# HuttleyLab/DiverseSeq

Measured on NVIDIA B200. Metric: prep_nmost_throughput, higher is better.
Workload: dtype u8 bases -> u32 counts -> f64 frequencies/entropy/JSD

## Files before the change

### diverseseq_b200/csrc/count.cu

```cuda
#include <stdlib.h>

#include <algorithm>

#include <functional>

#include "comm.cuh"
#include "common.cuh"
#include "fused.cuh"
#include "entropy.cuh"

namespace dvs {

struct CountWork {
    uint64_t begin;
    uint64_t end;
    uint32_t rec;
    uint32_t part;
};

constexpr int kCountThreads = 512;
constexpr int kPrefetch = 4;

__device__ __forceinline__ uint32_t pack4(uint32_t w) {
    return (w * 0x40100401u) >> 24;
}
__device__ __forceinline__ uint32_t pack16(uint4 v) {
    return (pack4(v.x) << 24) | (pack4(v.y) << 16) | (pack4(v.z) << 8) | pack4(v.w);
}

__device__ __forceinline__ uint4 ldg16(const uint8_t* p) { return __ldg(reinterpret_cast<const uint4*>(p)); }

template <bool SMEM>
__global__ void __launch_bounds__(kCountThreads)
k_count_generic(const uint8_t* __restrict__ seqs, const uint64_t* __restrict__ offsets,
                const CountWork* __restrict__ work, uint32_t nwork, uint32_t* __restrict__ next_item, int k,
                uint32_t num_states, uint64_t dim, uint32_t part_bins, uint32_t* __restrict__ counts) {
    extern __shared__ uint32_t hist[];
    __shared__ uint32_t s_item;
    const int tid = threadIdx.x;
    for (;;) {
        if (tid == 0) s_item = atomicAdd(next_item, 1u);
        __syncthreads();
        const uint32_t item = s_item;
        if (item >= nwork) break;
        const CountWork w = work[item];
        const uint64_t start = offsets[w.rec], end = offsets[w.rec + 1];
        const uint32_t part_base = w.part * part_bins;
        uint32_t* grow = counts + (size_t)w.rec * dim;
        if (SMEM) {
            for (uint32_t i = tid; i < part_bins; i += kCountThreads) hist[i] = 0;
            __syncthreads();
        }
        for (uint64_t a = w.begin + (uint64_t)tid * 16; a < w.end; a += (uint64_t)kCountThreads * 16) {
            const uint4 cur = ldg16(seqs + a);
            const uint4 prev = ldg16(seqs + a - 16);
            const uint32_t wv[8] = {prev.x, prev.y, prev.z, prev.w, cur.x, cur.y, cur.z, cur.w};
            uint32_t run = 0;
            uint64_t idx = 0;
#pragma unroll
            for (int i = 0; i < 32; ++i) {
                const uint64_t p = a - 16 + i;
                uint32_t b = (wv[i >> 2] >> (8 * (i & 3))) & 0xFFu;
                if (p < start || p >= end) b = 0xFFu;
                if (b >= num_states) {
                    run = 0;
                    idx = 0;
                } else {
                    idx = (idx * num_states + b) % dim;
                    ++run;
                    if (i >= 16 && run >= (uint32_t)k) {
                        if (SMEM) {
                            uint32_t local = (uint32_t)idx - part_base;
                            if (local < part_bins) atomicAdd(&hist[local], 1u);
                        } else {
                            atomicAdd(&grow[idx], 1u);
                        }
                    }
                }
            }
        }
        if (SMEM) {
            __syncthreads();
            for (uint32_t i = tid; i < part_bins; i += kCountThreads) {
                uint32_t c = hist[i];
                if (c && (uint64_t)part_base + i < dim) atomicAdd(&grow[part_base + i], c);
            }
        }
        __syncthreads();
    }
}

constexpr int MODE_SMEM = 0, MODE_SMEM_PARTS = 1, MODE_GLOBAL = 2, MODE_SUPER = 3, MODE_SUPER3 = 4;

__device__ __forceinline__ uint32_t pack16p(uint4 v) {
    const uint32_t p0 = v.x * 0x40100401u, p1 = v.y * 0x40100401u, p2 = v.z * 0x40100401u, p3 = v.w * 0x40100401u;
    const uint32_t hi = __byte_perm(p1, p0, 0x7300);
    const uint32_t lo = __byte_perm(p3, p2, 0x0073);
    return __byte_perm(lo, hi, 0x7610);
}

__device__ __forceinline__ uint32_t scr_word(uint32_t idx) { return idx ^ (idx >> 5); }

template <int MODE, bool SCR, int THREADS>
__global__ void __launch_bounds__(THREADS)
k_count(const uint8_t* __restrict__ seqs, const uint64_t* __restrict__ offsets, const CountWork* __restrict__ work,
        uint32_t nwork, uint32_t* __restrict__ next_item, int k, uint64_t dim, uint32_t part_bins,
        uint32_t* __restrict__ counts, const uint32_t* __restrict__ nwork_dev) {
    extern __shared__ uint32_t hist[];
    __shared__ uint32_t s_item;
    if (nwork_dev) nwork = *nwork_dev;
    const int tid = threadIdx.x, lane = tid & 31, warp = tid >> 5;
    constexpr int kWarps = THREADS / 32;
    constexpr uint32_t kFull = 0xffffffffu;
    const int kk = (MODE == MODE_SUPER) ? k + 1 : k;
    const uint32_t mask = (kk >= 16) ? 0xFFFFFFFFu : ((1u << (2 * kk)) - 1u);
    const uint32_t mask4 = mask << 2;
    const uint32_t mask_k = (k >= 16) ? 0xFFFFFFFFu : ((1u << (2 * k)) - 1u);
    const uint32_t hist_words = (MODE == MODE_SUPER) ? (uint32_t)(dim * 4 + dim)
                                                     : (MODE == MODE_SMEM_PARTS ? part_bins + 1 : part_bins);
    uint32_t* side = hist + dim * 4;
    char* const hist_b = reinterpret_cast<char*>(hist);

    for (;;) {
        if (tid == 0) s_item = atomicAdd(next_item, 1u);
        __syncthreads();
        const uint32_t item = s_item;
        if (item >= nwork) break;
        const CountWork w = work[item];
        const uint64_t start = offsets[w.rec], end = offsets[w.rec + 1];
        const uint32_t part_base = (MODE == MODE_SMEM_PARTS) ? w.part * part_bins : 0u;
        uint32_t* grow = counts + (size_t)w.rec * dim;
        if (MODE != MODE_GLOBAL) {
            for (uint32_t i = tid; i < hist_words; i += THREADS) hist[i] = 0;
            __syncthreads();
        }
        auto bump4 = [&](uint32_t idx4) {
            if (MODE == MODE_SMEM || MODE == MODE_SUPER) {
                if (SCR) idx4 ^= (idx4 >> 5) & ~3u;
                atomicAdd(reinterpret_cast<uint32_t*>(hist_b + idx4), 1u);
            } else if (MODE == MODE_SMEM_PARTS) {
                uint32_t local4 = idx4 - (part_base << 2);
                if (SCR) local4 ^= (local4 >> 5) & ~3u;
                local4 = min(local4, part_bins << 2);
                atomicAdd(reinterpret_cast<uint32_t*>(hist_b + local4), 1u);
            } else {
                atomicAdd(&grow[idx4 >> 2], 1u);
            }
        };

        const uint32_t item_len = (uint32_t)(w.end - w.begin);
        const uint32_t rs = start > w.begin ? (uint32_t)min(start - w.begin, (uint64_t)item_len) : 0u;
        const uint32_t re = end < w.end ? (end > w.begin ? (uint32_t)(end - w.begin) : 0u) : item_len;
        const uint32_t span = ((item_len + kWarps - 1) / kWarps + 511u) & ~511u;
        const uint32_t r0 = min(item_len, (uint32_t)warp * span);
        const uint32_t r1 = min(item_len, r0 + span);
        const uint8_t* base = seqs + w.begin;
        uint32_t carry_pc = 0;
        bool carry_ok = false;
        uint4 ring[kPrefetch];
#pragma unroll
        for (int u = 0; u < kPrefetch; ++u) {
            const uint32_t a = r0 + 512u * u + 16 * lane;
            ring[u] = (a < r1) ? ldg16(base + a) : make_uint4(~0u, ~0u, ~0u, ~0u);
        }
        if (r0 < r1) {
            const uint4 h = ldg16(base + r0 - 16);
            const uint64_t a0 = w.begin + r0;
            carry_ok = (((h.x | h.y | h.z | h.w) & 0xFCFCFCFCu) == 0) && (a0 >= start + 16) && (a0 <= end);
            carry_pc = pack16p(h);
        }
        for (uint32_t rbase = r0; rbase < r1; rbase += 512u * kPrefetch) {
#pragma unroll
          for (int u = 0; u < kPrefetch; ++u) {
            const uint32_t r = rbase + 512u * u;
            if (r >= r1) break;
            const uint32_t a = r + 16 * lane;
            const uint4 cur = ring[u];
            ring[u] = (a + 512u * kPrefetch < r1) ? ldg16(base + a + 512u * kPrefetch) : make_uint4(~0u, ~0u, ~0u, ~0u);
            const bool ok = (((cur.x | cur.y | cur.z | cur.w) & 0xFCFCFCFCu) == 0) && (a >= rs) && (a + 16 <= re) && (a < r1);
            const uint32_t pc = pack16p(cur);
            uint32_t pp = __shfl_up_sync(kFull, pc, 1);
            if (lane == 0) pp = carry_pc;
            const uint32_t okmask = __ballot_sync(kFull, ok);
            const bool all_fast = (okmask == kFull) && carry_ok;
            if (all_fast) {
                if (MODE == MODE_SUPER) {
#pragma unroll
                    for (int j = 1; j < 15; j += 2) bump4(__funnelshift_r(pc, pp, 2 * (15 - j) - 2) & mask4);
                    bump4((pc << 2) & mask4);
                } else {
#pragma unroll
                    for (int j = 0; j < 15; ++j) bump4(__funnelshift_r(pc, pp, 2 * (15 - j) - 2) & mask4);
                    bump4((pc << 2) & mask4);
                }
            } else if (a < r1) {
                const bool prev_ok = lane == 0 ? carry_ok : ((okmask >> (lane - 1)) & 1u) != 0;
                if (ok && prev_ok) {
                    if (MODE == MODE_SUPER) {
#pragma unroll
                        for (int j = 1; j < 16; j += 2) bump4((__funnelshift_r(pc, pp, 2 * (15 - j)) & mask) << 2);
                    } else {
#pragma unroll
                        for (int j = 0; j < 16; ++j) bump4((__funnelshift_r(pc, pp, 2 * (15 - j)) & mask) << 2);
                    }
                } else {
                    const uint4 prev = ldg16(base + a - 16);
                    const uint32_t wv[8] = {prev.x, prev.y, prev.z, prev.w, cur.x, cur.y, cur.z, cur.w};
                    uint32_t run = 0, idx = 0, run_even = 0, idx_even = 0;
#pragma unroll
                    for (int i = 0; i < 32; ++i) {
                        const uint64_t p = w.begin + a + i - 16;
                        uint32_t bb = (wv[i >> 2] >> (8 * (i & 3))) & 0xFFu;
                        if (p < start || p >= end) bb = 0xFFu;
                        if (bb >= 4u) {
                            run = 0;
                            idx = 0;
                        } else {
                            idx = ((idx << 2) | bb) & mask;
                            ++run;
                        }
                        if (i < 16) continue;
                        if (MODE != MODE_SUPER) {
                            if (run >= (uint32_t)k) bump4(idx << 2);
                        } else if ((i & 1) == 0) {
                            run_even = run;
                            idx_even = idx;
                        } else if (run >= (uint32_t)(k + 1)) {
                            bump4(idx << 2);
                        } else {
                            if (run_even >= (uint32_t)k) atomicAdd(&side[idx_even & mask_k], 1u);
                            if (run >= (uint32_t)k) atomicAdd(&side[idx & mask_k], 1u);
                        }
                    }
                }
            }
            carry_pc = __shfl_sync(kFull, pc, 31);
            carry_ok = (okmask >> 31) != 0;
          }
        }
        if (MODE != MODE_GLOBAL) {
            __syncthreads();
            if (MODE == MODE_SUPER) {
                for (uint32_t x = tid; x < (uint32_t)dim; x += THREADS) {
                    uint32_t c = side[x];
#pragma unroll
                    for (uint32_t b = 0; b < 4; ++b) {
                        const uint32_t y = (x << 2) | b;
                        c += hist[SCR ? scr_word(y) : y];
                    }
#pragma unroll
                    for (uint32_t a4 = 0; a4 < 4; ++a4) {
                        const uint32_t y = (a4 << (2 * k)) | x;
                        c += hist[SCR ? scr_word(y) : y];
                    }
                    if (c) atomicAdd(&grow[x], c);
                }
            } else {
                for (uint32_t i = tid; i < part_bins; i += THREADS) {
                    uint32_t c = hist[SCR ? scr_word(i) : i];
                    if (c && (uint64_t)part_base + i < dim) atomicAdd(&grow[part_base + i], c);
                }
            }
        }
        __syncthreads();
    }
}

__device__ __forceinline__ void ldg32(const uint8_t* p, uint32_t (&v)[8]) {
    asm volatile("ld.global.nc.v8.u32 {%0,%1,%2,%3,%4,%5,%6,%7}, [%8];"
                 : "=r"(v[0]), "=r"(v[1]), "=r"(v[2]), "=r"(v[3]), "=r"(v[4]), "=r"(v[5]), "=r"(v[6]), "=r"(v[7])
                 : "l"(p));
}
__device__ __forceinline__ uint32_t pack16w(uint32_t x, uint32_t y, uint32_t z, uint32_t w) {
    return pack16p(make_uint4(x, y, z, w));
}

template <bool SCR, int THREADS, int PF>
__device__ __forceinline__ void
count_s3_body(const uint8_t* __restrict__ seqs, const uint64_t* __restrict__ offsets, const CountWork* __restrict__ work,
           uint32_t nwork, uint32_t* __restrict__ next_item, int k, uint64_t dim, uint32_t* __restrict__ counts,
           CountWork* __restrict__ retry, uint32_t* __restrict__ retry_count, uint32_t* resident) {
    extern __shared__ uint32_t hist[];
    __shared__ uint32_t s_item, s_sum, s_inc;
    if (resident && threadIdx.x == 0) atomicAdd(resident, 1u);
    const int tid = threadIdx.x, lane = tid & 31, warp = tid >> 5;
    constexpr int kWarps = THREADS / 32;
    constexpr uint32_t kFull = 0xffffffffu, kStep = 1024u;
    const int kk = k + 2;
    const uint32_t mask = (1u << (2 * kk)) - 1u;
    const uint32_t mask_k = (1u << (2 * k)) - 1u;
    const uint32_t hwords = (uint32_t)(dim * 8);
    uint32_t* side = hist + hwords;
    char* const hist_b = reinterpret_cast<char*>(hist);
    char* const side_b = reinterpret_cast<char*>(side);
    const uint32_t offmask = mask << 1 & ~3u, sidemask4 = mask_k << 2;
    const uint32_t lane32 = 32u * (uint32_t)lane;

    for (;;) {
        if (tid == 0) {
            s_item = atomicAdd(next_item, 1u);
            s_sum = 0;
            s_inc = 0;
        }
        __syncthreads();
        const uint32_t item = s_item;
        if (item >= nwork) break;
        const CountWork w = work[item];
        const uint64_t start = offsets[w.rec], end = offsets[w.rec + 1];
        uint32_t* grow = counts + (size_t)w.rec * dim;
        {
            uint4* h4 = reinterpret_cast<uint4*>(hist);
            const uint32_t n4 = (hwords + (uint32_t)dim) / 4;
            for (uint32_t i = tid; i < n4; i += THREADS) h4[i] = make_uint4(0, 0, 0, 0);
        }
        __syncthreads();
        uint32_t n_fast = 0;
        auto bump_v = [&](uint32_t v) {
            uint32_t off = v & offmask;
            if (SCR) off ^= (off >> 5) & ~3u;
            atomicAdd(reinterpret_cast<uint32_t*>(hist_b + off), (v & 2u) ? 0x10000u : 1u);
        };
        auto fast_block = [&](uint32_t pc, uint32_t pp) {
#pragma unroll
            for (int t = 0; t < 5; ++t) bump_v(__funnelshift_r(pc, pp, 25 - 6 * t));
            atomicAdd(reinterpret_cast<uint32_t*>(side_b + ((pc << 2) & sidemask4)), 1u);
        };

        const uint32_t item_len = (uint32_t)(w.end - w.begin);
        const uint32_t rs = start > w.begin ? (uint32_t)min(start - w.begin, (uint64_t)item_len) : 0u;
        const uint32_t re = end < w.end ? (end > w.begin ? (uint32_t)(end - w.begin) : 0u) : item_len;
        const uint32_t span = ((item_len + kWarps - 1) / kWarps + kStep - 1u) & ~(kStep - 1u);
        const uint32_t r0 = min(item_len, (uint32_t)warp * span);
        const uint32_t r1 = min(item_len, r0 + span);
        const uint8_t* base = seqs + w.begin;
        const uint32_t safe_hi = min(re, r1);
        uint32_t carry_pc = 0;
        bool carry_ok = false;
        uint32_t ring[PF][8];
#pragma unroll
        for (int u = 0; u < PF; ++u) {
            const uint32_t a = r0 + kStep * u + lane32;
            if (a < r1) ldg32(base + a, ring[u]);
            else {
#pragma unroll
                for (int q = 0; q < 8; ++q) ring[u][q] = ~0u;
            }
        }
        if (r0 < r1) {
            const uint4 h = ldg16(base + r0 - 16);
            const uint64_t a0 = w.begin + r0;
            carry_ok = (((h.x | h.y | h.z | h.w) & 0xFCFCFCFCu) == 0) && (a0 >= start + 16) && (a0 <= end);
            carry_pc = pack16p(h);
        }
        for (uint32_t rbase = r0; rbase < r1; rbase += kStep * PF) {
#pragma unroll
          for (int u = 0; u < PF; ++u) {
            const uint32_t r = rbase + kStep * u;
            if (r >= r1) break;
            const uint32_t a = r + lane32;
            uint32_t any = ring[u][0] | ring[u][1] | ring[u][2] | ring[u][3] | ring[u][4] | ring[u][5] | ring[u][6] | ring[u][7];
            bool ok = (any & 0xFCFCFCFCu) == 0;
            if (!(r >= rs && r + kStep <= safe_hi)) ok = ok && (a >= rs) && (a + 32 <= safe_hi);
            const uint32_t pc0 = pack16w(ring[u][0], ring[u][1], ring[u][2], ring[u][3]);
            const uint32_t pc1 = pack16w(ring[u][4], ring[u][5], ring[u][6], ring[u][7]);
            {
                const uint32_t an = a + kStep * PF;
                if (an < r1) ldg32(base + an, ring[u]);
                else {
#pragma unroll
                    for (int q = 0; q < 8; ++q) ring[u][q] = ~0u;
                }
            }
            uint32_t pp0 = __shfl_up_sync(kFull, pc1, 1);
            if (lane == 0) pp0 = carry_pc;
            const uint32_t okmask = __ballot_sync(kFull, ok);
            bool fast = okmask == kFull && carry_ok;
            if (!fast) {
                const bool prev_ok = lane == 0 ? carry_ok : ((okmask >> (lane - 1)) & 1u) != 0;
                fast = ok && prev_ok;
            }
            if (fast) {
                fast_block(pc0, pp0);
                fast_block(pc1, pc0);
                n_fast += 2;
            } else if (a < r1) {
                const uint4 q0 = ldg16(base + a - 16), q1 = ldg16(base + a), q2 = ldg16(base + a + 16);
                const uint32_t wv[12] = {q0.x, q0.y, q0.z, q0.w, q1.x, q1.y, q1.z, q1.w, q2.x, q2.y, q2.z, q2.w};
                uint32_t run = 0, idx = 0;
#pragma unroll 4
                for (int i = 0; i < 48; ++i) {
                    const uint64_t p = w.begin + a + i - 16;
                    uint32_t bb = (wv[i >> 2] >> (8 * (i & 3))) & 0xFFu;
                    if (p < start || p >= end) bb = 0xFFu;
                    if (bb >= 4u) {
                        run = 0;
                        idx = 0;
                    } else {
                        idx = ((idx << 2) | bb) & mask_k;
                        ++run;
                        if (i >= 16 && a + i - 16 < r1 && run >= (uint32_t)k) atomicAdd(&side[idx], 1u);
                    }
                }
            }
            carry_pc = __shfl_sync(kFull, pc1, 31);
            carry_ok = (okmask >> 31) != 0;
          }
        }
        __syncthreads();
        uint32_t pre_sum = 0;
        auto word_at = [&](uint32_t wd) { return hist[SCR ? (wd ^ (wd >> 5)) : wd]; };
        for (uint32_t x = tid; x < (uint32_t)dim; x += THREADS) {
            uint32_t c = side[x], pre = 0;
#pragma unroll
            for (uint32_t t = 0; t < 8; ++t) {
                const uint32_t v = word_at((x << 3) | t);
                pre += (v & 0xFFFFu) + (v >> 16);
            }
            c += pre;
            pre_sum += pre;
#pragma unroll
            for (uint32_t a4 = 0; a4 < 4; ++a4) {
#pragma unroll
                for (uint32_t t = 0; t < 2; ++t) {
                    const uint32_t v = word_at((a4 << (2 * k + 1)) | (x << 1) | t);
                    c += (v & 0xFFFFu) + (v >> 16);
                }
            }
#pragma unroll
            for (uint32_t t = 0; t < 16; ++t) {
                const uint32_t v = word_at((t << (2 * k - 1)) | (x >> 1));
                c += (x & 1u) ? (v >> 16) : (v & 0xFFFFu);
            }
            side[x] = c;
        }
        uint32_t n_inc = 5u * n_fast;
#pragma unroll
        for (int o = 16; o; o >>= 1) {
            pre_sum += __shfl_xor_sync(kFull, pre_sum, o);
            n_inc += __shfl_xor_sync(kFull, n_inc, o);
        }
        if (lane == 0) {
            atomicAdd(&s_sum, pre_sum);
            atomicAdd(&s_inc, n_inc);
        }
        __syncthreads();
        if (s_sum == s_inc) {
            for (uint32_t x = tid; x < (uint32_t)dim; x += THREADS) {
                const uint32_t c = side[x];
                if (c) atomicAdd(&grow[x], c);
            }
        } else if (tid == 0) {
            retry[atomicAdd(retry_count, 1u)] = w;
        }
        __syncthreads();
    }
    if (resident && threadIdx.x == 0) atomicSub(resident, 1u);
}

template <bool SCR, int THREADS, int PF>
__global__ void __launch_bounds__(THREADS, 1)
k_count_s3(const uint8_t* __restrict__ seqs, const uint64_t* __restrict__ offsets, const CountWork* __restrict__ work,
           uint32_t nwork, uint32_t* __restrict__ next_item, int k, uint64_t dim, uint32_t* __restrict__ counts,
           CountWork* __restrict__ retry, uint32_t* __restrict__ retry_count) {
    count_s3_body<SCR, THREADS, PF>(seqs, offsets, work, nwork, next_item, k, dim, counts, retry, retry_count, nullptr);
}
template <int MAXR>
__global__ void __maxnreg__(MAXR)
k_count_s3_trail(const uint8_t* __restrict__ seqs, const uint64_t* __restrict__ offsets,
                 const CountWork* __restrict__ work, uint32_t nwork, uint32_t* __restrict__ next_item, int k,
                 uint64_t dim, uint32_t* __restrict__ counts, CountWork* __restrict__ retry,
                 uint32_t* __restrict__ retry_count, uint32_t* resident) {
    count_s3_body<false, 1024, 2>(seqs, offsets, work, nwork, next_item, k, dim, counts, retry, retry_count, resident);
}

__global__ void __launch_bounds__(kEntThreads)
k_freq_entropy(const uint32_t* __restrict__ counts, uint64_t dim, double* __restrict__ freqs,
               uint64_t* __restrict__ totals, double* __restrict__ entropy, uint8_t* __restrict__ valid,
               uint8_t* __restrict__ err, double* __restrict__ err_total, const uint32_t* __restrict__ rec_list) {
    extern __shared__ __align__(16) double ent_smem[];
    __shared__ unsigned long long s_total;
    const uint32_t r = rec_list ? rec_list[blockIdx.x] : blockIdx.x;
    const uint32_t* c = counts + (size_t)r * dim;
    double* f = freqs + (size_t)r * dim;
    if (threadIdx.x == 0) s_total = 0ULL;
    __syncthreads();
    unsigned long long part = 0;
    for (uint64_t i = threadIdx.x; i < dim; i += blockDim.x) part += c[i];
    for (int o = 16; o; o >>= 1) part += __shfl_xor_sync(0xffffffffu, part, o);
    if ((threadIdx.x & 31) == 0) atomicAdd(&s_total, part);
    __syncthreads();
    const unsigned long long total_u = s_total;
    const double total = (double)total_u;
    if (total_u == 0ULL) {
        for (uint64_t i = threadIdx.x; i < dim; i += blockDim.x) f[i] = __ddiv_rn((double)c[i], total);
        if (threadIdx.x == 0) {
            totals[r] = 0;
            entropy[r] = 0.0;
            valid[r] = 0;
            err[r] = 0;
            err_total[r] = 0.0;
        }
        return;
    }
    const FastDiv dv = make_fast_div(total);
    EntropyResult h = block_entropy_exact(dim, [&](uint64_t i) {
        const double x = div_exact((double)c[i], dv);
        f[i] = x;
        return x;
    }, ent_smem);
    if (threadIdx.x == 0) {
        totals[r] = total_u;
        entropy[r] = h.e;
        valid[r] = 1;
        bool bad = entropy_total_bad(h.t, dim);
        err[r] = bad ? 1 : 0;
        err_total[r] = h.t;
    }
}

__global__ void __launch_bounds__(kEntThreads)
k_rows_entropy(const double* __restrict__ freqs, uint64_t dim, double* __restrict__ entropy,
               uint8_t* __restrict__ err, double* __restrict__ err_total, int write_entropy) {
    extern __shared__ __align__(16) double ent_smem[];
    const uint32_t r = blockIdx.x;
    const double* f = freqs + (size_t)r * dim;
    EntropyResult h = block_entropy_exact(dim, [&](uint64_t i) { return f[i]; }, ent_smem);
    if (threadIdx.x == 0) {
        if (write_entropy) entropy[r] = h.e;
        bool bad = entropy_total_bad(h.t, dim);
        err[r] = bad ? 1 : 0;
        err_total[r] = h.t;
    }
}

__global__ void k_take_rows(const double* __restrict__ F, const double* __restrict__ H, const uint8_t* __restrict__ V,
                            const uint8_t* __restrict__ E, const double* __restrict__ ET, uint64_t dim,
                            const uint32_t* __restrict__ rows, double* __restrict__ Fo, double* __restrict__ Ho,
                            uint8_t* __restrict__ Vo, uint8_t* __restrict__ Eo, double* __restrict__ ETo) {
    const uint32_t i = blockIdx.x, r = rows[i];
    const double* src = F + (size_t)r * dim;
    double* dst = Fo + (size_t)i * dim;
    for (uint64_t c = threadIdx.x; c < dim; c += blockDim.x) dst[c] = src[c];
    if (threadIdx.x == 0) {
        Ho[i] = H[r];
        Vo[i] = V[r];
        Eo[i] = E[r];
        ETo[i] = ET[r];
    }
}

__global__ void k_log2(const double* x, double* y, uint64_t n) {
    uint64_t i = (uint64_t)blockIdx.x * blockDim.x + threadIdx.x;
    if (i < n) y[i] = dvs_log2(x[i]);
}

static bool pow_dim(int num_states, int k, uint64_t* dim) {
    uint64_t d = 1;
    for (int i = 0; i < k; ++i) {
        d *= (uint64_t)num_states;
        if (d > (1ULL << 32)) return false;
    }
    *dim = d;
    return true;
}

static int kfreqs_alloc(dvs_ctx* ctx, uint32_t nrec, uint64_t dim, bool with_counts, dvs_kfreqs** out) {
    DVS_CUDA_TRY(dvs::enter(ctx));
    auto* f = new dvs_kfreqs();
    f->device = ctx->device;
    f->nrec = nrec;
    f->dim = dim;
    f->has_counts = with_counts;
    int rc = DVS_OK;
    if (with_counts) rc = f->counts.alloc((size_t)nrec * dim);
    if (rc == DVS_OK) rc = f->freqs.alloc((size_t)nrec * dim);
    if (rc == DVS_OK) rc = f->totals.alloc(nrec);
    if (rc == DVS_OK) rc = f->entropy.alloc(nrec);
    if (rc == DVS_OK) rc = f->valid.alloc(nrec);
    if (rc == DVS_OK) rc = f->err.alloc(nrec);
    if (rc == DVS_OK) rc = f->err_total.alloc(nrec);
    if (rc != DVS_OK) {
        delete f;
        return rc;
    }
    *out = f;
    return DVS_OK;
}

}

using namespace dvs;

extern "C" {

struct CountDest {
    double* freqs;
    uint64_t* totals;
    double* entropy;
    uint8_t* valid;
    uint8_t* err;
    double* err_total;
    uint32_t chunks;
    std::function<int(uint32_t, uint32_t)> after_chunk;
    const uint32_t* rec_seq = nullptr;
    int s3_shape = -1;
    uint32_t* resident = nullptr;
    int trail_regs = 56;
    const uint32_t* weights = nullptr;
};

static int count_core(dvs_ctx* ctx, const dvs_seqset* s, int k, int num_states, uint32_t* d_counts, uint64_t dim,
                      const CountDest& dst) {
    cudaStream_t st = ctx->stream;
#define TRY_F(expr)                                                          \
    do {                                                                     \
        cudaError_t _e = (expr);                                             \
        if (_e != cudaSuccess) {                                             \
            set_error("%s failed: %s", #expr, cudaGetErrorString(_e));       \
            return DVS_ERR_CUDA;                                             \
        }                                                                    \
    } while (0)

    TRY_F(cudaMemsetAsync(d_counts, 0, (size_t)s->nrec * dim * sizeof(uint32_t), st));

    const bool ns4 = (num_states == 4);
    const size_t max_hist_bytes = std::min<size_t>(ctx->smem_optin > 4096 ? ctx->smem_optin - 2048 : 0, 128 * 1024 + 16);
    uint32_t nparts = 1, part_bins = (uint32_t)std::min<uint64_t>(dim, 1u << 31);
    int mode = MODE_SMEM;
    size_t hist_bytes = (size_t)dim * 4;
    const char* s3_env = getenv("DVS_COUNT_S3");
    const bool want_s3 = !(s3_env && s3_env[0] == '0');
    if (ns4 && want_s3 && k >= 4 && dim * 36 + 2048 <= ctx->smem_optin && dim * 36 <= 160 * 1024) {
        mode = MODE_SUPER3;
        hist_bytes = (size_t)dim * 36;
    } else if (ns4 && dim * 20 <= 96 * 1024) {
        mode = MODE_SUPER;
        hist_bytes = (size_t)dim * 20;
    } else if (dim * 4 > max_hist_bytes) {
        uint64_t bins_per = max_hist_bytes / 4;
        uint64_t np = (dim + bins_per - 1) / bins_per;
        if (np <= 2) {
            mode = MODE_SMEM_PARTS;
            nparts = (uint32_t)np;
            part_bins = (uint32_t)((dim + np - 1) / np);
            hist_bytes = (size_t)part_bins * 4 + 16;
        } else {
            mode = MODE_GLOBAL;
            hist_bytes = 0;
        }
    }
    const bool smem = (mode != MODE_GLOBAL);
    const char* scr_env = getenv("DVS_COUNT_SCRAMBLE");
    const bool scramble = !(scr_env && scr_env[0] == '0');

    int ctas_per_sm = 4;
    if (smem) ctas_per_sm = (int)std::max<size_t>(1, std::min<size_t>(4, (ctx->smem_optin + 1024) / (hist_bytes + 1024)));
    const uint32_t grid = (uint32_t)(ctx->sm_count * ctas_per_sm);
    const int threads4 = (mode == MODE_SMEM_PARTS || mode == MODE_SUPER3) ? 1024 : kCountThreads;
    uint64_t chunk = 1 << 20;
    {
        const uint64_t flush_bins =
            (mode == MODE_GLOBAL) ? 0 : (mode == MODE_SUPER ? dim : (mode == MODE_SUPER3 ? dim * 16 : part_bins));
        const uint64_t max_chunk = flush_bins >= 32768 ? (8u << 20) : (flush_bins >= 16384 ? (2u << 20) : (1u << 20));
        uint64_t want_items = (uint64_t)grid * 8 * dst.chunks;
        uint64_t c = (s->total + want_items - 1) / std::max<uint64_t>(want_items, 1);
        c = std::max<uint64_t>(64 << 10, std::min<uint64_t>(c, max_chunk));
        chunk = (c + 8191) / 8192 * 8192;
        if (mode == MODE_GLOBAL && dim * 4 >= (16u << 20)) chunk = 8192;
    }
    DevBuf<uint32_t> d_rec_seq;
    if (dst.rec_seq) {
        if (d_rec_seq.alloc(std::max<uint32_t>(s->nrec, 1)) != DVS_OK) return DVS_ERR_CUDA;
        TRY_F(cudaMemcpyAsync(d_rec_seq.p, dst.rec_seq, (size_t)s->nrec * sizeof(uint32_t), cudaMemcpyHostToDevice, st));
    }
    const bool same_seq = dst.rec_seq ? (s->work_seq.size() == s->nrec &&
                                         std::equal(s->work_seq.begin(), s->work_seq.end(), dst.rec_seq))
                                      : s->work_seq.empty();
    if (s->work_chunk != chunk || s->work_nparts != nparts || !s->work_cache.p || !same_seq) {
        std::vector<CountWork> work;
        s->work_item_begin.assign(s->nrec + 1, 0);
        for (uint32_t q = 0; q < s->nrec; ++q) {
            const uint32_t r = dst.rec_seq ? dst.rec_seq[q] : q;
            s->work_item_begin[q] = (uint32_t)work.size();
            uint64_t b = s->h_offsets[r], e = s->h_offsets[r + 1];
            if (e <= b) continue;
            uint64_t a0 = b & ~31ULL, a1 = (e + 15) & ~15ULL;
            for (uint64_t a = a0; a < a1; a += chunk)
                for (uint32_t p = 0; p < nparts; ++p) work.push_back({a, std::min(a + chunk, a1), r, p});
        }
        if (work.size() > 0xFFFFFFF0ull) {
            dvs::set_error("too many counting work items");
            return DVS_ERR_ARG;
        }
        s->work_item_begin[s->nrec] = (uint32_t)work.size();
        s->work_chunk = 0;
        if (s->work_cache.alloc(work.size() * sizeof(CountWork)) != DVS_OK) return DVS_ERR_CUDA;
        TRY_F(cudaMemcpyAsync(s->work_cache.p, work.data(), work.size() * sizeof(CountWork), cudaMemcpyHostToDevice, st));
        s->work_chunk = chunk;
        s->work_nparts = nparts;
        s->work_items = (uint32_t)work.size();
        if (dst.rec_seq)
            s->work_seq.assign(dst.rec_seq, dst.rec_seq + s->nrec);
        else
            s->work_seq.clear();
    }
    const CountWork* d_work_all = reinterpret_cast<const CountWork*>(s->work_cache.p);
    const uint32_t nchunks = std::max<uint32_t>(1, std::min<uint32_t>(dst.chunks, std::max<uint32_t>(s->nrec, 1)));
    DevBuf<uint32_t> d_next, d_rc;
    DevBuf<CountWork> d_retry;
    if (d_next.alloc(nchunks) != DVS_OK) return DVS_ERR_CUDA;
    TRY_F(cudaMemsetAsync(d_next.p, 0, nchunks * sizeof(uint32_t), st));
    if (mode == MODE_SUPER3) {
        if (d_retry.alloc(std::max<uint32_t>(s->work_items, 1)) != DVS_OK || d_rc.alloc(2 * nchunks) != DVS_OK)
            return DVS_ERR_CUDA;
        TRY_F(cudaMemsetAsync(d_rc.p, 0, 2 * nchunks * sizeof(uint32_t), st));
    }
    PhaseTimer pt_all(nchunks > 1 ? ctx : nullptr, DVS_PHASE_COUNT_KERNEL);
    struct TimingGuard {
        dvs_ctx* c;
        bool saved;
        ~TimingGuard() { c->timing = saved; }
    } timing_guard{ctx, ctx->timing};
    if (nchunks > 1) ctx->timing = false;
    const bool chunk_ev = nchunks > 1 && timing_guard.saved && nchunks <= 64;
    ctx->n_chunk_ev = 0;
    if (chunk_ev)
        for (uint32_t i = 0; i < 2 * nchunks; ++i)
            if (!ctx->ev_chunk[i]) TRY_F(cudaEventCreate(&ctx->ev_chunk[i]));
    uint64_t wsum = 0;
    for (uint32_t c = 0; c < nchunks && dst.weights; ++c) wsum += dst.weights[c];
    auto chunk_first = [&](uint32_t c) -> uint32_t {
        if (!dst.weights || !wsum) return (uint32_t)((uint64_t)s->nrec * c / nchunks);
        uint64_t acc = 0;
        for (uint32_t i = 0; i < c; ++i) acc += dst.weights[i];
        return (uint32_t)((unsigned __int128)s->nrec * acc / wsum);
    };
    for (uint32_t ch = 0; ch < nchunks; ++ch) {
        const uint32_t rb = chunk_first(ch), re = chunk_first(ch + 1);
        const uint32_t ib = s->work_item_begin[rb], ie = s->work_item_begin[re];
        const CountWork* d_work = d_work_all + ib;
        const uint32_t n_work = ie - ib;
        uint32_t* d_nx = d_next.p + ch;
        if (n_work) {
            const uint32_t g = (uint32_t)std::min<size_t>(grid, n_work);
            auto set_smem = [&](auto kern) -> cudaError_t {
                return hist_bytes > 48 * 1024
                           ? cudaFuncSetAttribute(kern, cudaFuncAttributeMaxDynamicSharedMemorySize, (int)hist_bytes)
                           : cudaSuccess;
            };
            auto launch4 = [&](auto kern) -> cudaError_t {
                cudaError_t e = set_smem(kern);
                if (e != cudaSuccess) return e;
                kern<<<g, threads4, hist_bytes, st>>>(s->data(), s->offsets.p, d_work, n_work, d_nx, k, dim, part_bins,
                                                      d_counts, nullptr);
                ctx->launches++;
                return cudaGetLastError();
            };
            auto launch_generic = [&](auto kern) -> cudaError_t {
                cudaError_t e = set_smem(kern);
                if (e != cudaSuccess) return e;
                kern<<<g, kCountThreads, hist_bytes, st>>>(s->data(), s->offsets.p, d_work, n_work, d_nx, k,
                                                           (uint32_t)num_states, dim, part_bins, d_counts);
                ctx->launches++;
                return cudaGetLastError();
            };
            cudaError_t e;
            PhaseTimer pt(ctx, DVS_PHASE_COUNT_KERNEL);
            if (chunk_ev) cudaEventRecord(ctx->ev_chunk[2 * ctx->n_chunk_ev], st);
            if (!ns4)
                e = smem ? launch_generic(k_count_generic<true>) : launch_generic(k_count_generic<false>);
            else if (mode == MODE_SUPER3) {
                const bool scr3 = scr_env && scr_env[0] == '1';
                const char* shape_env = getenv("DVS_COUNT_S3_SHAPE");
                const int shape = dst.s3_shape >= 0 ? dst.s3_shape : (shape_env ? atoi(shape_env) : 0);
                auto s3 = scr3 ? k_count_s3<true, 1024, 2>
                               : (shape == 1 ? k_count_s3<false, 1024, 2>
                                             : (shape == 2 ? k_count_s3<false, 512, 4> : k_count_s3<false, 1024, 3>));
                const int s3_threads = (!scr3 && shape == 2) ? 512 : 1024;
                auto rk = scramble ? k_count<MODE_SUPER, true, 512> : k_count<MODE_SUPER, false, 512>;
                const char* pad_env = getenv("DVS_COUNT_SMEM_PAD");
                const size_t s3_bytes = hist_bytes + (pad_env ? (size_t)atoi(pad_env) : 0);
                TRY_F(cudaFuncSetAttribute(s3, cudaFuncAttributeMaxDynamicSharedMemorySize, (int)s3_bytes));
                const size_t retry_bytes = (size_t)dim * 20;
                if (retry_bytes > 48 * 1024)
                    TRY_F(cudaFuncSetAttribute(rk, cudaFuncAttributeMaxDynamicSharedMemorySize, (int)retry_bytes));
                uint32_t* rc2 = d_rc.p + 2 * ch;
                if (dst.resident) {
                    auto k_count_s3_trail = dst.trail_regs <= 40 ? dvs::k_count_s3_trail<40>
                                            : (dst.trail_regs <= 48 ? dvs::k_count_s3_trail<48> : dvs::k_count_s3_trail<56>);
                    TRY_F(cudaFuncSetAttribute(k_count_s3_trail, cudaFuncAttributeMaxDynamicSharedMemorySize, (int)s3_bytes));
                    TRY_F(cudaFuncSetAttribute(k_count_s3_trail, cudaFuncAttributePreferredSharedMemoryCarveout,
                                               (int)cudaSharedmemCarveoutMaxShared));
                    k_count_s3_trail<<<g, 1024, s3_bytes, st>>>(s->data(), s->offsets.p, d_work, n_work, d_nx, k, dim,
                                                                d_counts, d_retry.p + ib, rc2, dst.resident);
                } else {
                    s3<<<g, s3_threads, s3_bytes, st>>>(s->data(), s->offsets.p, d_work, n_work, d_nx, k, dim, d_counts,
                                                        d_retry.p + ib, rc2);
                }
                ctx->launches++;
                e = cudaGetLastError();
                if (e == cudaSuccess) {
                    const uint32_t g2 = (uint32_t)std::min<size_t>((size_t)ctx->sm_count * 2, n_work);
                    rk<<<g2, 512, retry_bytes, st>>>(s->data(), s->offsets.p, d_retry.p + ib, 0u, rc2 + 1, k, dim,
                                                     (uint32_t)dim, d_counts, rc2);
                    ctx->launches++;
                    e = cudaGetLastError();
                }
            } else if (mode == MODE_SUPER)
                e = scramble ? launch4(k_count<MODE_SUPER, true, 512>) : launch4(k_count<MODE_SUPER, false, 512>);
            else if (mode == MODE_SMEM)
                e = scramble ? launch4(k_count<MODE_SMEM, true, 512>) : launch4(k_count<MODE_SMEM, false, 512>);
            else if (mode == MODE_SMEM_PARTS)
                e = scramble ? launch4(k_count<MODE_SMEM_PARTS, true, 1024>) : launch4(k_count<MODE_SMEM_PARTS, false, 1024>);
            else
                e = launch4(k_count<MODE_GLOBAL, false, 512>);
            pt.stop();
            if (chunk_ev) cudaEventRecord(ctx->ev_chunk[2 * ctx->n_chunk_ev++ + 1], st);
            if (e != cudaSuccess) {
                set_error("k_count launch failed: %s", cudaGetErrorString(e));
                return DVS_ERR_CUDA;
            }
        }
        if (re > rb) {
            PhaseTimer pt(ctx, DVS_PHASE_FREQ_ENTROPY);
            if (dst.rec_seq)
                k_freq_entropy<<<re - rb, kEntThreads, kEntSmemBytes, st>>>(d_counts, dim, dst.freqs, dst.totals, dst.entropy,
                                                                            dst.valid, dst.err, dst.err_total, d_rec_seq.p + rb);
            else
                k_freq_entropy<<<re - rb, kEntThreads, kEntSmemBytes, st>>>(
                    d_counts + (size_t)rb * dim, dim, dst.freqs + (size_t)rb * dim, dst.totals + rb, dst.entropy + rb,
                    dst.valid + rb, dst.err + rb, dst.err_total + rb, nullptr);
            ctx->launches++;
            TRY_F(cudaGetLastError());
        }
        if (dst.after_chunk) DVS_TRY(dst.after_chunk(rb, re));
    }
    ctx->timing = timing_guard.saved;
    pt_all.stop();
#undef TRY_F
    return DVS_OK;
}

static int count_args_ok(dvs_ctx* ctx, const dvs_seqset* s, int k, int num_states, const void* out, uint64_t* dim) {
    if (!ctx || !s || !out) {
        set_error("dvs_count_kmers: NULL argument");
        return DVS_ERR_ARG;
    }
    if (k == 0) {
        set_error("k cannot be 0");
        return DVS_ERR_VALUE;
    }
    if (k < 0 || k > 16 || num_states < 1 || num_states > 255) {
        set_error("dvs_count_kmers: unsupported k=%d / num_states=%d (need 1<=k<=16, 1<=num_states<=255)", k,
                  num_states);
        return DVS_ERR_ARG;
    }
    if (!pow_dim(num_states, k, dim)) {
        set_error("dvs_count_kmers: num_states^k = %d^%d does not fit a dense u32-indexed table", num_states, k);
        return DVS_ERR_ARG;
    }
    for (uint32_t r = 0; r < s->nrec; ++r)
        if (s->h_offsets[r + 1] - s->h_offsets[r] >= (1ULL << 32)) {
            set_error("dvs_count_kmers: record %u has %llu bases; records of 2^32 bases or more are not supported "
                      "(32-bit bin counters)", r, (unsigned long long)(s->h_offsets[r + 1] - s->h_offsets[r]));
            return DVS_ERR_ARG;
        }
    return DVS_OK;
}

static int dense_rows_fit(double need, const char* what, uint32_t nrec, uint64_t dim) {
    size_t free_b = 0, total_b = 0;
    if (need > 8e9) DVS_CUDA_TRY(cudaMemGetInfo(&free_b, &total_b));
    if (need > 8e9 && need > 0.9 * (double)free_b) {
        set_error("%s: dense rows need %.1f GB (nrec=%u, dim=%llu) but only %.1f GB are free", what, need / 1e9, nrec,
                  (unsigned long long)dim, free_b / 1e9);
        return DVS_ERR_ARG;
    }
    return DVS_OK;
}

int dvs_count_kmers(dvs_ctx* ctx, const dvs_seqset* s, int k, int num_states, dvs_kfreqs** out) {
    uint64_t dim = 0;
    DVS_TRY(count_args_ok(ctx, s, k, num_states, out, &dim));
    DVS_CUDA_TRY(dvs::enter(ctx));
    DVS_TRY(dense_rows_fit((double)s->nrec * (double)dim * 12.0, "dvs_count_kmers", s->nrec, dim));
    dvs_kfreqs* f = nullptr;
    DVS_TRY(kfreqs_alloc(ctx, s->nrec, dim, true, &f));
    f->k = k;
    f->num_states = num_states;
    CountDest dst{f->freqs.p, f->totals.p, f->entropy.p, f->valid.p, f->err.p, f->err_total.p, 1, nullptr};
    int rc = count_core(ctx, s, k, num_states, f->counts.p, dim, dst);
    if (rc != DVS_OK) {
        dvs_kfreqs_free(f);
        return rc;
    }
    *out = f;
    return DVS_OK;
}

__global__ void k_set_word(unsigned* w, unsigned v) { *w = v; }

int dvs_count_select(dvs_ctx* ctx, const dvs_seqset* s, int k, int num_states, const uint32_t* order, uint32_t num,
                     int mode, uint32_t min_size, uint32_t max_size, uint32_t chunks, dvs_kfreqs** out,
                     uint32_t* sel_idx, double* sel_delta, double* stats5, uint32_t* size_out) {
    uint64_t dim = 0;
    DVS_TRY(count_args_ok(ctx, s, k, num_states, out, &dim));
    if ((!order && num) || !size_out) {
        set_error("dvs_count_select: NULL argument");
        return DVS_ERR_ARG;
    }
    for (uint32_t i = 0; i < num; ++i)
        if (order[i] >= s->nrec) {
            set_error("dvs_count_select: order[%u]=%u out of range (nrec=%u)", i, order[i], s->nrec);
            return DVS_ERR_ARG;
        }
    DVS_CUDA_TRY(dvs::enter(ctx));
    DVS_TRY(dense_rows_fit((double)s->nrec * (double)dim * 12.0, "dvs_count_select", s->nrec, dim));
    if (!ctx->stream2) {
        DVS_CUDA_TRY(cudaStreamCreateWithFlags(&ctx->stream2, cudaStreamNonBlocking));
        DVS_CUDA_TRY(cudaEventCreateWithFlags(&ctx->ev_first, cudaEventDisableTiming));
        DVS_CUDA_TRY(cudaEventCreateWithFlags(&ctx->ev_count_done, cudaEventDisableTiming));
        DVS_CUDA_TRY(cudaEventCreateWithFlags(&ctx->ev_fork, cudaEventDisableTiming));
        DVS_CUDA_TRY(cudaMalloc(&ctx->d_ready, 4096));
    }
    dvs_kfreqs* f = nullptr;
    DVS_TRY(kfreqs_alloc(ctx, s->nrec, dim, true, &f));
    f->k = k;
    f->num_states = num_states;

    std::vector<uint32_t> seq, seqpos(s->nrec, 0xFFFFFFFFu);
    seq.reserve(s->nrec);
    for (uint32_t i = 0; i < num; ++i)
        if (seqpos[order[i]] == 0xFFFFFFFFu) {
            seqpos[order[i]] = (uint32_t)seq.size();
            seq.push_back(order[i]);
        }
    for (uint32_t r = 0; r < s->nrec; ++r)
        if (seqpos[r] == 0xFFFFFFFFu) {
            seqpos[r] = (uint32_t)seq.size();
            seq.push_back(r);
        }
    std::vector<uint32_t> need(num);
    for (uint32_t i = 0, m = 0; i < num; ++i) {
        m = std::max(m, seqpos[order[i]] + 1);
        need[i] = m;
    }
    auto ready_after = [&](uint32_t re) {
        return (uint32_t)(std::upper_bound(need.begin(), need.end(), re) - need.begin());
    };
    std::vector<uint32_t> weights;
    if (const char* w_env = getenv("DVS_TRAIL_WEIGHTS")) {
        for (const char* p = w_env; *p;) {
            char* end = nullptr;
            const unsigned long v = strtoul(p, &end, 10);
            if (end == p) break;
            weights.push_back((uint32_t)std::max<unsigned long>(v, 1));
            p = *end ? end + 1 : end;
        }
        if (weights.size() >= 2 && weights.size() <= 64) chunks = (uint32_t)weights.size();
        else weights.clear();
    }
    if (chunks == 0 && weights.empty()) {
        weights = {3, 4, 4, 3, 2, 1};
        chunks = 6;
    }
    chunks = std::min<uint32_t>(chunks, 64);
    auto first_chunk_end = [&]() -> uint32_t {
        if (weights.size() != chunks) return (uint32_t)((uint64_t)s->nrec / chunks);
        uint64_t ws = 0;
        for (uint32_t w : weights) ws += w;
        return (uint32_t)((uint64_t)s->nrec * weights[0] / ws);
    };
    while (chunks > 1 && ready_after(first_chunk_end()) < std::max<uint32_t>(min_size, 1)) {
        --chunks;
        weights.clear();
    }
    const char* s3_env = getenv("DVS_COUNT_S3");
    const bool s3 = num_states == 4 && k >= 4 && k <= 6 && !(s3_env && s3_env[0] == '0');
    const bool trail = chunks > 1 && mode == DVS_MODE_NMOST && num > 0 && s3;
    const char* trail_env = getenv("DVS_TRAIL");
    const bool trail_rounds = !(trail_env && trail_env[0] == '0');

    cudaStream_t main_st = ctx->stream;
    int rc;
    if (!trail) {
        CountDest dst{f->freqs.p, f->totals.p, f->entropy.p, f->valid.p, f->err.p, f->err_total.p, 1, nullptr};
        rc = count_core(ctx, s, k, num_states, f->counts.p, dim, dst);
        if (rc == DVS_OK)
            rc = dvs::select_with_trail(ctx, f, order, num, mode, min_size, max_size, sel_idx, sel_delta, stats5,
                                        size_out, nullptr);
    } else {
        dvs::TrailArgs ta{ctx->d_ready, 0, ctx->ev_first, ctx->ev_count_done, ctx->d_ready + 1};
        DVS_CUDA_TRY(cudaMemsetAsync(ctx->d_ready, 0, 8, main_st));
        DVS_CUDA_TRY(cudaEventRecord(ctx->ev_fork, main_st));
        DVS_CUDA_TRY(cudaStreamWaitEvent(ctx->stream2, ctx->ev_fork, 0));
        CountDest dst{f->freqs.p, f->totals.p, f->entropy.p, f->valid.p, f->err.p, f->err_total.p, chunks, nullptr};
        dst.rec_seq = seq.data();
        if (weights.size() == chunks) dst.weights = weights.data();
        if (dvs::trail_shape() != 3) {
            dst.s3_shape = 1;
            dst.resident = ctx->d_ready + 1;
            dst.trail_regs = dvs::trail_count_regs();
        }
        bool first = true;
        cudaStream_t side = ctx->stream2;
        dst.after_chunk = [&](uint32_t, uint32_t re) -> int {
            const uint32_t rdy = ready_after(re);
            k_set_word<<<1, 1, 0, side>>>(ctx->d_ready, rdy);
            DVS_CUDA_TRY(cudaGetLastError());
            if (first) {
                first = false;
                ta.limit0 = rdy;
                DVS_CUDA_TRY(cudaEventRecord(ctx->ev_first, side));
            }
            return DVS_OK;
        };
        ctx->stream = side;
        dvs::tl_stream = side;
        rc = count_core(ctx, s, k, num_states, f->counts.p, dim, dst);
        cudaError_t e1 = first ? cudaEventRecord(ctx->ev_first, side) : cudaSuccess;
        cudaError_t e2 = cudaEventRecord(ctx->ev_count_done, side);
        ctx->stream = main_st;
        dvs::tl_stream = main_st;
        if (rc == DVS_OK && (e1 != cudaSuccess || e2 != cudaSuccess)) {
            set_error("dvs_count_select: cudaEventRecord failed");
            rc = DVS_ERR_CUDA;
        }
        if (rc == DVS_OK && !trail_rounds) cudaStreamWaitEvent(main_st, ctx->ev_count_done, 0);
        if (rc == DVS_OK)
            rc = dvs::select_with_trail(ctx, f, order, num, mode, min_size, max_size, sel_idx, sel_delta, stats5,
                                        size_out, trail_rounds ? &ta : nullptr);
        cudaStreamWaitEvent(main_st, ctx->ev_count_done, 0);
        if (getenv("DVS_TRAIL_DEBUG") && ctx->timing) {
            cudaStreamSynchronize(main_st);
            fprintf(stderr, "[dvs] count launches (ms):");
            for (uint32_t c = 0; c < ctx->n_chunk_ev; ++c) {
                float ms = 0.f;
                cudaEventElapsedTime(&ms, ctx->ev_chunk[2 * c], ctx->ev_chunk[2 * c + 1]);
                fprintf(stderr, " %.3f", ms);
            }
            fprintf(stderr, "  trailing launches %u, fewest SMs %u, accepts while counting %u\n", ctx->last_trail_launches,
                    ctx->last_trail_launches ? ctx->last_trail_sms : 0, ctx->last_trail_accepts);
        }
    }
    if (rc != DVS_OK) {
        cudaStreamSynchronize(main_st);
        dvs_kfreqs_free(f);
        return rc;
    }
    *out = f;
    return DVS_OK;
}

struct AllRows {
    dvs_kfreqs* f = nullptr;
    uint64_t off_freqs = 0, off_ent = 0, off_et = 0, off_tot = 0, off_valid = 0, off_err = 0;
    uint32_t row0 = 0, total = 0;
};

static int allrows_alloc(dvs_ctx* ctx, dvs_comm* c, const uint32_t* nrec_per_rank, uint64_t dim, AllRows* a) {
    uint64_t total = 0;
    for (int r = 0; r < c->world; ++r) {
        if (r == c->rank) a->row0 = (uint32_t)total;
        total += nrec_per_rank[r];
    }
    if (total > 0xFFFFFFF0ull) {
        set_error("too many records in total");
        return DVS_ERR_ARG;
    }
    a->total = (uint32_t)total;
    auto up = [](uint64_t x) { return (x + 255) & ~255ull; };
    const uint64_t n = std::max<uint64_t>(total, 1);
    a->off_freqs = 0;
    a->off_ent = up(n * dim * 8);
    a->off_et = a->off_ent + up(n * 8);
    a->off_tot = a->off_et + up(n * 8);
    a->off_valid = a->off_tot + up(n * 8);
    a->off_err = a->off_valid + up(n);
    const uint64_t bytes = a->off_err + up(n);
    uint64_t hoff = 0;
    DVS_TRY(comm_heap_alloc(c, bytes, &hoff));
    auto* f = new dvs_kfreqs();
    f->device = ctx->device;
    f->nrec = a->total;
    f->dim = dim;
    f->has_counts = false;
    f->heap = c;
    f->heap_off = hoff;
    uint8_t* base = c->window + hoff;
    f->freqs.borrow(reinterpret_cast<double*>(base + a->off_freqs), n * dim);
    f->entropy.borrow(reinterpret_cast<double*>(base + a->off_ent), n);
    f->err_total.borrow(reinterpret_cast<double*>(base + a->off_et), n);
// ... 341 lines not shown
```

Measured before the change: 3419.

## Replace per-16-mer side atomics with packed (k+1)-mer pair histogram for k>=5

Reworks the fast counting path of the super3 k-mer counter so that each 32-base piece issues one packed 16-bit atomic into a new (k+1)-mer pair histogram instead of two side-table atomics, when k>=5. The reduction phase then recovers the missing k-mers from the pair histogram. This cuts shared-memory atomics per piece and adjusts the increment count. In exchange the per-bin shared footprint grows from 36 to 44 bytes, which can exclude some k from the S3 path or lower occupancy, and the reduction does more reads.

```diff
diff --git a/diverseseq_b200/csrc/count.cu b/diverseseq_b200/csrc/count.cu
--- a/diverseseq_b200/csrc/count.cu
+++ b/diverseseq_b200/csrc/count.cu
@@ -3,6 +3,7 @@
 #include <algorithm>
 
 #include <functional>
+#include <type_traits>
 
 #include "comm.cuh"
 #include "common.cuh"
@@ -275,7 +276,8 @@
     return pack16p(make_uint4(x, y, z, w));
 }
 
-template <bool SCR, int THREADS, int PF>
+inline bool s3_pair(int k) { return k >= 5; }
+template <bool SCR, int THREADS, int PF, bool PAIR>
 __device__ __forceinline__ void
 count_s3_body(const uint8_t* __restrict__ seqs, const uint64_t* __restrict__ offsets, const CountWork* __restrict__ work,
            uint32_t nwork, uint32_t* __restrict__ next_item, int k, uint64_t dim, uint32_t* __restrict__ counts,
@@ -291,9 +293,11 @@
     const uint32_t mask_k = (1u << (2 * k)) - 1u;
     const uint32_t hwords = (uint32_t)(dim * 8);
     uint32_t* side = hist + hwords;
+    const uint32_t* pair = side + dim;
     char* const hist_b = reinterpret_cast<char*>(hist);
+    char* const pair_b = reinterpret_cast<char*>(side + dim);
     char* const side_b = reinterpret_cast<char*>(side);
-    const uint32_t offmask = mask << 1 & ~3u, sidemask4 = mask_k << 2;
+    const uint32_t offmask = mask << 1 & ~3u, poffmask = ((mask_k << 2) | 3u) << 1 & ~3u, sidemask4 = mask_k << 2;
     const uint32_t lane32 = 32u * (uint32_t)lane;
 
     for (;;) {
@@ -310,20 +314,28 @@
         uint32_t* grow = counts + (size_t)w.rec * dim;
         {
             uint4* h4 = reinterpret_cast<uint4*>(hist);
-            const uint32_t n4 = (hwords + (uint32_t)dim) / 4;
+            const uint32_t n4 = (hwords + (PAIR ? 3u : 1u) * (uint32_t)dim) / 4;
             for (uint32_t i = tid; i < n4; i += THREADS) h4[i] = make_uint4(0, 0, 0, 0);
         }
         __syncthreads();
-        uint32_t n_fast = 0;
+        uint32_t n_inc = 0;
         auto bump_v = [&](uint32_t v) {
             uint32_t off = v & offmask;
             if (SCR) off ^= (off >> 5) & ~3u;
             atomicAdd(reinterpret_cast<uint32_t*>(hist_b + off), (v & 2u) ? 0x10000u : 1u);
         };
-        auto fast_block = [&](uint32_t pc, uint32_t pp) {
-#pragma unroll
-            for (int t = 0; t < 5; ++t) bump_v(__funnelshift_r(pc, pp, 25 - 6 * t));
-            atomicAdd(reinterpret_cast<uint32_t*>(side_b + ((pc << 2) & sidemask4)), 1u);
+        auto fast_piece = [&](uint32_t pp0, uint32_t pc0, uint32_t pc1) {
+#pragma unroll
+            for (int t = 0; t < 5; ++t) bump_v(__funnelshift_r(pc0, pp0, 25 - 6 * t));
+#pragma unroll
+            for (int t = 0; t < 5; ++t) bump_v(__funnelshift_r(pc1, pc0, 27 - 6 * t));
+            if (PAIR) {
+                const uint32_t v = pc1 << 1;
+                atomicAdd(reinterpret_cast<uint32_t*>(pair_b + (v & poffmask)), (v & 2u) ? 0x10000u : 1u);
+            } else {
+                atomicAdd(reinterpret_cast<uint32_t*>(side_b + (pc1 & sidemask4)), 1u);
+                atomicAdd(reinterpret_cast<uint32_t*>(side_b + ((pc1 << 2) & sidemask4)), 1u);
+            }
         };
 
         const uint32_t item_len = (uint32_t)(w.end - w.begin);
@@ -380,9 +392,8 @@
                 fast = ok && prev_ok;
             }
             if (fast) {
-                fast_block(pc0, pp0);
-                fast_block(pc1, pc0);
-                n_fast += 2;
+                fast_piece(pp0, pc0, pc1);
+                n_inc += PAIR ? 11u : 10u;
             } else if (a < r1) {
                 const uint4 q0 = ldg16(base + a - 16), q1 = ldg16(base + a), q2 = ldg16(base + a + 16);
                 const uint32_t wv[12] = {q0.x, q0.y, q0.z, q0.w, q1.x, q1.y, q1.z, q1.w, q2.x, q2.y, q2.z, q2.w};
@@ -416,6 +427,18 @@
                 const uint32_t v = word_at((x << 3) | t);
                 pre += (v & 0xFFFFu) + (v >> 16);
             }
+            if (PAIR) {
+#pragma unroll
+                for (uint32_t t = 0; t < 2; ++t) {
+                    const uint32_t v = pair[(x << 1) | t];
+                    pre += (v & 0xFFFFu) + (v >> 16);
+                }
+#pragma unroll
+                for (uint32_t a4 = 0; a4 < 4; ++a4) {
+                    const uint32_t v = pair[(a4 << (2 * k - 1)) | (x >> 1)];
+                    c += (x & 1u) ? (v >> 16) : (v & 0xFFFFu);
+                }
+            }
             c += pre;
             pre_sum += pre;
 #pragma unroll
@@ -433,7 +456,6 @@
             }
             side[x] = c;
         }
-        uint32_t n_inc = 5u * n_fast;
 #pragma unroll
         for (int o = 16; o; o >>= 1) {
             pre_sum += __shfl_xor_sync(kFull, pre_sum, o);
@@ -457,20 +479,20 @@
     if (resident && threadIdx.x == 0) atomicSub(resident, 1u);
 }
 
-template <bool SCR, int THREADS, int PF>
+template <bool SCR, int THREADS, int PF, bool PAIR>
 __global__ void __launch_bounds__(THREADS, 1)
 k_count_s3(const uint8_t* __restrict__ seqs, const uint64_t* __restrict__ offsets, const CountWork* __restrict__ work,
            uint32_t nwork, uint32_t* __restrict__ next_item, int k, uint64_t dim, uint32_t* __restrict__ counts,
            CountWork* __restrict__ retry, uint32_t* __restrict__ retry_count) {
-    count_s3_body<SCR, THREADS, PF>(seqs, offsets, work, nwork, next_item, k, dim, counts, retry, retry_count, nullptr);
-}
-template <int MAXR>
+    count_s3_body<SCR, THREADS, PF, PAIR>(seqs, offsets, work, nwork, next_item, k, dim, counts, retry, retry_count, nullptr);
+}
+template <int MAXR, bool PAIR>
 __global__ void __maxnreg__(MAXR)
 k_count_s3_trail(const uint8_t* __restrict__ seqs, const uint64_t* __restrict__ offsets,
                  const CountWork* __restrict__ work, uint32_t nwork, uint32_t* __restrict__ next_item, int k,
                  uint64_t dim, uint32_t* __restrict__ counts, CountWork* __restrict__ retry,
                  uint32_t* __restrict__ retry_count, uint32_t* resident) {
-    count_s3_body<false, 1024, 2>(seqs, offsets, work, nwork, next_item, k, dim, counts, retry, retry_count, resident);
+    count_s3_body<false, 1024, 2, PAIR>(seqs, offsets, work, nwork, next_item, k, dim, counts, retry, retry_count, resident);
 }
 
 __global__ void __launch_bounds__(kEntThreads)
@@ -630,9 +652,10 @@
     size_t hist_bytes = (size_t)dim * 4;
     const char* s3_env = getenv("DVS_COUNT_S3");
     const bool want_s3 = !(s3_env && s3_env[0] == '0');
-    if (ns4 && want_s3 && k >= 4 && dim * 36 + 2048 <= ctx->smem_optin && dim * 36 <= 160 * 1024) {
+    const uint64_t s3_per_bin = s3_pair(k) ? 44 : 36;
+    if (ns4 && want_s3 && k >= 4 && dim * s3_per_bin + 2048 <= ctx->smem_optin && dim * s3_per_bin <= 180 * 1024) {
         mode = MODE_SUPER3;
-        hist_bytes = (size_t)dim * 36;
+        hist_bytes = (size_t)(dim * s3_per_bin);
     } else if (ns4 && dim * 20 <= 96 * 1024) {
         mode = MODE_SUPER;
         hist_bytes = (size_t)dim * 20;
@@ -773,9 +796,13 @@
                 const bool scr3 = scr_env && scr_env[0] == '1';
                 const char* shape_env = getenv("DVS_COUNT_S3_SHAPE");
                 const int shape = dst.s3_shape >= 0 ? dst.s3_shape : (shape_env ? atoi(shape_env) : 0);
-                auto s3 = scr3 ? k_count_s3<true, 1024, 2>
-                               : (shape == 1 ? k_count_s3<false, 1024, 2>
-                                             : (shape == 2 ? k_count_s3<false, 512, 4> : k_count_s3<false, 1024, 3>));
+                auto pick_s3 = [&](auto pair_c) {
+                    constexpr bool P = decltype(pair_c)::value;
+                    return scr3 ? k_count_s3<true, 1024, 2, P>
+                                : (shape == 1 ? k_count_s3<false, 1024, 2, P>
+                                              : (shape == 2 ? k_count_s3<false, 512, 4, P> : k_count_s3<false, 1024, 3, P>));
+                };
+                auto s3 = s3_pair(k) ? pick_s3(std::true_type{}) : pick_s3(std::false_type{});
                 const int s3_threads = (!scr3 && shape == 2) ? 512 : 1024;
                 auto rk = scramble ? k_count<MODE_SUPER, true, 512> : k_count<MODE_SUPER, false, 512>;
                 const char* pad_env = getenv("DVS_COUNT_SMEM_PAD");
@@ -786,8 +813,13 @@
                     TRY_F(cudaFuncSetAttribute(rk, cudaFuncAttributeMaxDynamicSharedMemorySize, (int)retry_bytes));
                 uint32_t* rc2 = d_rc.p + 2 * ch;
                 if (dst.resident) {
-                    auto k_count_s3_trail = dst.trail_regs <= 40 ? dvs::k_count_s3_trail<40>
-                                            : (dst.trail_regs <= 48 ? dvs::k_count_s3_trail<48> : dvs::k_count_s3_trail<56>);
+                    auto pick_trail = [&](auto pair_c) {
+                        constexpr bool P = decltype(pair_c)::value;
+                        return dst.trail_regs <= 40 ? dvs::k_count_s3_trail<40, P>
+                                                    : (dst.trail_regs <= 48 ? dvs::k_count_s3_trail<48, P>
+                                                                            : dvs::k_count_s3_trail<56, P>);
+                    };
+                    auto k_count_s3_trail = s3_pair(k) ? pick_trail(std::true_type{}) : pick_trail(std::false_type{});
                     TRY_F(cudaFuncSetAttribute(k_count_s3_trail, cudaFuncAttributeMaxDynamicSharedMemorySize, (int)s3_bytes));
                     TRY_F(cudaFuncSetAttribute(k_count_s3_trail, cudaFuncAttributePreferredSharedMemoryCarveout,
                                                (int)cudaSharedmemCarveoutMaxShared));
```

Result: faster. 3464 (median of 6 runs) (+1.3%).
